# wdmwhh/MRefSR

Measured on AMD Instinct MI355X. Metric: 4x SR Mpix/sec, 5-ref 160x160->640x640; PSNR within 0.01 dB of ref, higher is better.
Workload: dtype f32

## Files before the change

### mrefsr_amd/csrc/mrattn_conv.hip

```cpp
#include "conv_common.h"

namespace {
using namespace mrefsr_conv;

constexpr int TG = 5;
constexpr int TR = 8, TW = 32;
constexpr int PH = TR + 2, PW = TW + 2, NPIX = PH * PW;
constexpr int QPL = NPIX * 16;
constexpr int TPL = 4 * QPL;
constexpr int NPIECE = NPIX * 4;
constexpr int NPK = (NPIECE + 255) / 256;
constexpr int NJ = 4;
constexpr int LDS_RAW = TG * TPL;
constexpr int LDS_BYTES = LDS_RAW + TR * TW * 4 + 64 + 16;

struct BlendArgs {
    const float *refs, *prob, *bias, *in_amax;
    const unsigned short *wp;
    const unsigned int *valid_bits;
    int *range_flag;
    float *out;
    int N, T, H, W, ncb;
    float out_scale;
};

template <int C, bool MASKED>
__global__ __launch_bounds__(256) void mrattn_blend_conv_kernel(const BlendArgs A)
{
    constexpr int NCH = C / KC, COUT = 2 * C, TAPS = 9, NW = 3;
    extern __shared__ __align__(16) unsigned char smem[];
    float *psum = reinterpret_cast<float *>(smem + LDS_RAW);
    int *tlist = reinterpret_cast<int *>(smem + LDS_RAW + TR * TW * 4);
    const int tid = threadIdx.x, lane = tid & 63, wv = tid >> 6, l31 = lane & 31, kh = lane >> 5;
    const int H = A.H, W = A.W, T = A.T, N = A.N;
    const int tx_n = (W + TW - 1) / TW, ty_n = (H + TR - 1) / TR;
    const unsigned int lin = blockIdx.x, seq = lin >> 3;
    const int cbk = (int)(seq % (unsigned)A.ncb);
    const long tile = (long)(seq / (unsigned)A.ncb) * 8 + (lin & 7u);
    if (tile >= (long)tx_n * ty_n * N) return;
    const int n = (int)(tile / (tx_n * ty_n)), trem = (int)(tile - (long)n * (tx_n * ty_n));
    const int y0 = (trem / tx_n) * TR, x0 = (trem % tx_n) * TW;

    if (tid == 0) {
        const unsigned int vb = MASKED ? A.valid_bits[n] : 0xffffffffu;
        int c = 0;
        for (int t = 0; t < T; ++t)
            if ((vb >> t) & 1u) tlist[c++] = t;
        tlist[16] = c;
    }
    float in_s = 1.f, oscale = A.out_scale;
    amax_scale<14>(A.in_amax, in_s, oscale);
    __syncthreads();
    const int total = __builtin_amdgcn_readfirstlane(tlist[16]);
    const int n_grp = (total + TG - 1) / TG, n_it = NCH * n_grp;

    const float *prow[2];
    bool pok[2];
#pragma unroll
    for (int m = 0; m < 2; ++m) {
        const int gy = y0 + wv * 2 + m, gx = x0 + l31;
        pok[m] = gy < H && gx < W;
        prow[m] = A.prob + (((size_t)n * H + (gy < H ? gy : H - 1)) * W + (gx < W ? gx : W - 1)) * T;
        float s = 0.f;
        for (int k = 0; k < total; ++k) s += prow[m][__builtin_amdgcn_readfirstlane(tlist[k])];
        if (kh == 0) psum[(wv * 2 + m) * TW + l31] = pok[m] ? s : 0.f;
    }

    f32x16 acc[2][NJ];
#pragma unroll
    for (int m = 0; m < 2; ++m)
#pragma unroll
        for (int j = 0; j < NJ; ++j)
#pragma unroll
            for (int e = 0; e < 16; ++e) acc[m][j][e] = 0.f;

    int goff[NPK], loff[NPK];
    unsigned int in_map = 0u, in_tile = 0u;
#pragma unroll
    for (int k = 0; k < NPK; ++k) {
        const int i = tid + k * 256;
        const int p = i >> 2, q = i & 3;
        const int py = p / PW, px = p - py * PW;
        const int gy = y0 + py - 1, gx = x0 + px - 1;
        const bool tile = i < NPIECE, ok = tile && gy >= 0 && gy < H && gx >= 0 && gx < W;
        goff[k] = ok ? (gy * W + gx) * C + 4 * q : 0;
        loff[k] = q * QPL + p * 16;
        in_map |= (ok ? 1u : 0u) << k, in_tile |= (tile ? 1u : 0u) << k;
    }
    float4 pf[TG][NPK];
    auto fetch = [&](const int it) {
        const int ch = it / n_grp, g = it - ch * n_grp;
        const int cnt = total - g * TG < TG ? total - g * TG : TG;
#pragma unroll
        for (int tg = 0; tg < TG; ++tg)
            if (tg < cnt) {
                const int t = __builtin_amdgcn_readfirstlane(tlist[g * TG + tg]);
                const float *base = A.refs + ((size_t)t * N + n) * H * W * C + ch * KC;
#pragma unroll
                for (int k = 0; k < NPK; ++k)
                    pf[tg][k] = ((in_map >> k) & 1u) ? *reinterpret_cast<const float4 *>(base + goff[k]) : make_float4(0.f, 0.f, 0.f, 0.f);
            }
    };
    if (n_it) fetch(0);

    const unsigned short *wlane = A.wp + (size_t)l31 * KC + kh * 8;
    auto bload = [&](const int lin, u32x4 (&b)[NJ][2]) {
#pragma unroll
        for (int j = 0; j < NJ; ++j)
#pragma unroll
            for (int sp = 0; sp < 2; ++sp)
                b[j][sp] = *reinterpret_cast<const u32x4 *>(wlane + ((((size_t)(cbk * 2 + (j >> 1)) * NCH * TAPS + lin) * NW + sp) * NB + (j & 1) * 32) * KC);
    };

    bool bad = false;
    float pr[2][TG];
    for (int it = 0; it < n_it; ++it) {
        const int ch = it / n_grp, g = it - ch * n_grp;
        const int cnt = total - g * TG < TG ? total - g * TG : TG;
        if (it) __syncthreads();
#pragma unroll
        for (int tg = 0; tg < TG; ++tg)
            if (tg < cnt) {
#pragma unroll
                for (int k = 0; k < NPK; ++k) {
                    float4 v = pf[tg][k];
                    v.x *= in_s, v.y *= in_s, v.z *= in_s, v.w *= in_s;
                    bad = bad || !(fmaxf(fmaxf(fabsf(v.x), fabsf(v.y)), fmaxf(fabsf(v.z), fabsf(v.w))) <= 65000.f);
                    if ((in_tile >> k) & 1u) *reinterpret_cast<float4 *>(smem + tg * TPL + loff[k]) = v;
                }
            }
        __syncthreads();
        if (it + 1 < n_it) fetch(it + 1);
        if (n_grp > 1 || it == 0) {
#pragma unroll
            for (int m = 0; m < 2; ++m)
#pragma unroll
                for (int k = 0; k < TG; ++k) pr[m][k] = (k < cnt && pok[m]) ? prow[m][__builtin_amdgcn_readfirstlane(tlist[g * TG + k])] : 0.f;
        }
        u32x4 b[NJ][2];
        bload(ch * TAPS, b);
#pragma nounroll
        for (int tap = 0; tap < TAPS; ++tap) {
            const int dy = (tap * 11) >> 5, dx = tap - 3 * dy;
            u32x4 bn[NJ][2];
            if (tap + 1 < TAPS) bload(ch * TAPS + tap + 1, bn);
#pragma unroll
            for (int m = 0; m < 2; ++m) {
                const unsigned char *sp = smem + (2 * kh) * QPL + ((wv * 2 + m + dy) * PW + l31 + dx) * 16;
                float u[8];
#pragma unroll
                for (int c = 0; c < 8; ++c) u[c] = 0.f;
#pragma unroll
                for (int k = 0; k < TG; ++k)
                    if (k < cnt) {
                        const float4 s0 = *reinterpret_cast<const float4 *>(sp + k * TPL);
                        const float4 s1 = *reinterpret_cast<const float4 *>(sp + k * TPL + QPL);
                        const float w = pr[m][k];
                        u[0] = fmaf(w, s0.x, u[0]), u[1] = fmaf(w, s0.y, u[1]), u[2] = fmaf(w, s0.z, u[2]), u[3] = fmaf(w, s0.w, u[3]);
                        u[4] = fmaf(w, s1.x, u[4]), u[5] = fmaf(w, s1.y, u[5]), u[6] = fmaf(w, s1.z, u[6]), u[7] = fmaf(w, s1.w, u[7]);
                    }
                u32x4 ah, al;
#pragma unroll
                for (int c = 0; c < 4; ++c) {
                    unsigned int h, l;
                    split_scaled(u[2 * c], u[2 * c + 1], h, l);
                    ah[c] = h, al[c] = l;
                }
#pragma unroll
                for (int j = 0; j < NJ; ++j) acc[m][j] = mma16(ah, b[j][1], acc[m][j]);
#pragma unroll
                for (int j = 0; j < NJ; ++j) acc[m][j] = mma16(al, scale_wh(b[j][0]), acc[m][j]);
#pragma unroll
                for (int j = 0; j < NJ; ++j) acc[m][j] = mma16(ah, b[j][0], acc[m][j]);
            }
            if (tap + 1 < TAPS) {
#pragma unroll
                for (int j = 0; j < NJ; ++j) b[j][0] = bn[j][0], b[j][1] = bn[j][1];
            }
        }
    }
    if (bad && A.range_flag) atomicOr(A.range_flag, 1);
    __syncthreads();

#pragma unroll
    for (int m = 0; m < 2; ++m) {
        const int gy = y0 + wv * 2 + m;
        if (gy >= H) continue;
#pragma unroll
        for (int j = 0; j < NJ; ++j) {
            const int co = cbk * (NJ * 32) + j * 32 + l31;
            const float bv = A.bias ? A.bias[co] : 0.f;
            float *orow = A.out + (((size_t)n * H + gy) * W) * COUT + co;
#pragma unroll
            for (int e = 0; e < 16; ++e) {
                const int x = (e & 3) + 8 * (e >> 2) + 4 * kh, gx = x0 + x;
                if (gx < W) orow[(size_t)gx * COUT] = acc[m][j][e] * oscale + bv * psum[(wv * 2 + m) * TW + x];
            }
        }
    }
}

template <int C, bool MASKED> int launch_blend_c(const BlendArgs &a, const dim3 grid, hipStream_t st)
{
    static unsigned long long attr_done = 0;
    if (mrefsr::first_use_on_device(attr_done)) {
        const hipError_t e = hipFuncSetAttribute(reinterpret_cast<const void *>(&mrattn_blend_conv_kernel<C, MASKED>),
                                                 hipFuncAttributeMaxDynamicSharedMemorySize, LDS_BYTES);
        if (e != hipSuccess) {
            attr_done = 0;
            (void)hipGetLastError();
            return mrefsr::fail(MREFSR_E_LAUNCH, "mrattn_blend_conv: %d bytes of dynamic LDS refused: %s", LDS_BYTES, hipGetErrorString(e));
        }
    }
    hipLaunchKernelGGL((mrattn_blend_conv_kernel<C, MASKED>), grid, dim3(256), LDS_BYTES, st, a);
    return mrefsr::check_launch("mrattn_blend_conv");
}

template <bool MASKED> int launch_blend(const BlendArgs &a, int C, hipStream_t st)
{
    const long tiles = (long)((a.W + TW - 1) / TW) * ((a.H + TR - 1) / TR) * a.N;
    const dim3 grid((unsigned)(((tiles + 7) / 8) * 8 * a.ncb));
    if (C == 64) return launch_blend_c<64, MASKED>(a, grid, st);
    if (C == 128) return launch_blend_c<128, MASKED>(a, grid, st);
    return launch_blend_c<256, MASKED>(a, grid, st);
}

}

MREFSR_EXPORT int mrefsr_mrattn_blend_conv_f32(const float *refs, const float *prob, const void *packed, const float *bias,
                                               const uint32_t *valid_bits, const float *in_amax, int *range_flag, float *out, int N, int T,
                                               int H, int W, int C, float wscale, mrefsr_stream_t stream)
{
    MREFSR_REQUIRE(refs && prob && packed && out, "mrattn_blend_conv: null pointer");
    MREFSR_REQUIRE(N > 0 && T > 0 && T <= 16 && H > 0 && W > 0, "mrattn_blend_conv: N=%d T=%d H=%d W=%d (T <= 16)", N, T, H, W);
    MREFSR_REQUIRE((int64_t)((W + TW - 1) / TW) * ((H + TR - 1) / TR) * N < (int64_t)1 << 28, "mrattn_blend_conv: N=%d H=%d W=%d (too many tiles)", N, H, W);
    MREFSR_REQUIRE((int64_t)H * W * 256 < (int64_t)1 << 31, "mrattn_blend_conv: H=%d W=%d (32-bit offsets inside a map)", H, W);
    MREFSR_REQUIRE(wscale > 0.f, "mrattn_blend_conv: wscale=%g", (double)wscale);
    if (C != 64 && C != 128 && C != 256)
        return mrefsr::fail(MREFSR_E_UNSUPPORTED, "mrattn_blend_conv: c=%d (64, 128 or 256: the three MRAPAFusion heads)", C);
    BlendArgs a;
    a.refs = refs, a.prob = prob, a.bias = bias, a.in_amax = in_amax;
    a.wp = reinterpret_cast<const unsigned short *>(packed);
    a.valid_bits = valid_bits, a.range_flag = range_flag, a.out = out;
    a.N = N, a.T = T, a.H = H, a.W = W, a.ncb = 2 * C / (NJ * 32);
    a.out_scale = 1.0f / wscale;
    return valid_bits ? launch_blend<true>(a, C, (hipStream_t)stream) : launch_blend<false>(a, C, (hipStream_t)stream);
}
```

Baseline: 17.25.

## Halve blend-conv tile rows, software-pipeline taps, and specialise on reference count

Tile height drops from 8 to 4 rows, so each wave handles one output row. Launch bounds now ask for two blocks per CU, with a static assert that LDS fits. The tap loop is fully unrolled and software-pipelined: the next tap's LDS reads, probability blend and hi/lo split are interleaved between the current tap's MFMAs using sched_barriers. The per-reference count is made a compile-time constant for 1 to 5 references. Input scaling moves into the probability weights, the range check becomes an integer max on the centre tap compared against a precomputed bound, and out-of-image halo is zeroed once rather than on every pass. The risks are more halo overhead per output pixel from the smaller tile, more register pressure, and rounding differences from folding the scale into the weights.

```diff
diff --git a/mrefsr_amd/csrc/mrattn_conv.hip b/mrefsr_amd/csrc/mrattn_conv.hip
--- a/mrefsr_amd/csrc/mrattn_conv.hip
+++ b/mrefsr_amd/csrc/mrattn_conv.hip
@@ -1,10 +1,12 @@
+#include <type_traits>
+
 #include "conv_common.h"
 
 namespace {
 using namespace mrefsr_conv;
 
 constexpr int TG = 5;
-constexpr int TR = 8, TW = 32;
+constexpr int TR = 4, TW = 32;
 constexpr int PH = TR + 2, PW = TW + 2, NPIX = PH * PW;
 constexpr int QPL = NPIX * 16;
 constexpr int TPL = 4 * QPL;
@@ -13,6 +15,7 @@
 constexpr int NJ = 4;
 constexpr int LDS_RAW = TG * TPL;
 constexpr int LDS_BYTES = LDS_RAW + TR * TW * 4 + 64 + 16;
+static_assert(2 * LDS_BYTES <= 160 * 1024, "two blocks per CU");
 
 struct BlendArgs {
     const float *refs, *prob, *bias, *in_amax;
@@ -25,7 +28,7 @@
 };
 
 template <int C, bool MASKED>
-__global__ __launch_bounds__(256) void mrattn_blend_conv_kernel(const BlendArgs A)
+__global__ __launch_bounds__(256, 2) void mrattn_blend_conv_kernel(const BlendArgs A)
 {
     constexpr int NCH = C / KC, COUT = 2 * C, TAPS = 9, NW = 3;
     extern __shared__ __align__(16) unsigned char smem[];
@@ -50,151 +53,180 @@
     }
     float in_s = 1.f, oscale = A.out_scale;
     amax_scale<14>(A.in_amax, in_s, oscale);
+    const unsigned int guard_bits = __float_as_uint(fminf(65000.f / in_s, 3.4028234664e38f));
     __syncthreads();
     const int total = __builtin_amdgcn_readfirstlane(tlist[16]);
     const int n_grp = (total + TG - 1) / TG, n_it = NCH * n_grp;
 
-    const float *prow[2];
-    bool pok[2];
-#pragma unroll
-    for (int m = 0; m < 2; ++m) {
-        const int gy = y0 + wv * 2 + m, gx = x0 + l31;
-        pok[m] = gy < H && gx < W;
-        prow[m] = A.prob + (((size_t)n * H + (gy < H ? gy : H - 1)) * W + (gx < W ? gx : W - 1)) * T;
+    const int gy_w = y0 + wv, gx_w = x0 + l31;
+    const bool pok = gy_w < H && gx_w < W;
+    const float *prow = A.prob + (((size_t)n * H + (gy_w < H ? gy_w : H - 1)) * W + (gx_w < W ? gx_w : W - 1)) * T;
+    {
         float s = 0.f;
-        for (int k = 0; k < total; ++k) s += prow[m][__builtin_amdgcn_readfirstlane(tlist[k])];
-        if (kh == 0) psum[(wv * 2 + m) * TW + l31] = pok[m] ? s : 0.f;
-    }
-
-    f32x16 acc[2][NJ];
-#pragma unroll
-    for (int m = 0; m < 2; ++m)
-#pragma unroll
-        for (int j = 0; j < NJ; ++j)
-#pragma unroll
-            for (int e = 0; e < 16; ++e) acc[m][j][e] = 0.f;
-
-    int goff[NPK], loff[NPK];
-    unsigned int in_map = 0u, in_tile = 0u;
+        for (int k = 0; k < total; ++k) s += prow[__builtin_amdgcn_readfirstlane(tlist[k])];
+        if (kh == 0) psum[wv * TW + l31] = pok ? s : 0.f;
+    }
+
+    f32x16 acc[NJ];
+#pragma unroll
+    for (int j = 0; j < NJ; ++j)
+#pragma unroll
+        for (int e = 0; e < 16; ++e) acc[j][e] = 0.f;
+
+    unsigned int goff[NPK], loff[NPK];
+    bool in_map[NPK];
 #pragma unroll
     for (int k = 0; k < NPK; ++k) {
         const int i = tid + k * 256;
         const int p = i >> 2, q = i & 3;
         const int py = p / PW, px = p - py * PW;
         const int gy = y0 + py - 1, gx = x0 + px - 1;
-        const bool tile = i < NPIECE, ok = tile && gy >= 0 && gy < H && gx >= 0 && gx < W;
-        goff[k] = ok ? (gy * W + gx) * C + 4 * q : 0;
-        loff[k] = q * QPL + p * 16;
-        in_map |= (ok ? 1u : 0u) << k, in_tile |= (tile ? 1u : 0u) << k;
-    }
-    float4 pf[TG][NPK];
-    auto fetch = [&](const int it) {
-        const int ch = it / n_grp, g = it - ch * n_grp;
-        const int cnt = total - g * TG < TG ? total - g * TG : TG;
-#pragma unroll
-        for (int tg = 0; tg < TG; ++tg)
-            if (tg < cnt) {
-                const int t = __builtin_amdgcn_readfirstlane(tlist[g * TG + tg]);
-                const float *base = A.refs + ((size_t)t * N + n) * H * W * C + ch * KC;
-#pragma unroll
-                for (int k = 0; k < NPK; ++k)
-                    pf[tg][k] = ((in_map >> k) & 1u) ? *reinterpret_cast<const float4 *>(base + goff[k]) : make_float4(0.f, 0.f, 0.f, 0.f);
+        const bool tile = i < NPIECE;
+        in_map[k] = tile && gy >= 0 && gy < H && gx >= 0 && gx < W;
+        goff[k] = in_map[k] ? (unsigned int)((gy * W + gx) * C + 4 * q) : 0u;
+        loff[k] = tile ? q * QPL + p * 16 : 0;
+        if (tile && !in_map[k]) {
+#pragma unroll
+            for (int tg = 0; tg < TG; ++tg) *reinterpret_cast<float4 *>(smem + tg * TPL + loff[k]) = make_float4(0.f, 0.f, 0.f, 0.f);
+        }
+    }
+
+    const unsigned int wl_off = (unsigned int)(l31 * KC + kh * 8) * 2u;
+    auto bload = [&](const int lin, u32x4 (&b)[NJ][2]) {
+#pragma unroll
+        for (int j = 0; j < NJ; ++j)
+#pragma unroll
+            for (int sp = 0; sp < 2; ++sp) {
+                const unsigned short *wu = A.wp + (((size_t)(cbk * 2 + (j >> 1)) * NCH * TAPS + lin) * NW * NB) * KC;
+                b[j][sp] = *reinterpret_cast<const u32x4 *>(reinterpret_cast<const unsigned char *>(wu) + wl_off + (sp * NB + (j & 1) * 32) * KC * 2);
             }
     };
-    if (n_it) fetch(0);
-
-    const unsigned short *wlane = A.wp + (size_t)l31 * KC + kh * 8;
-    auto bload = [&](const int lin, u32x4 (&b)[NJ][2]) {
-#pragma unroll
-        for (int j = 0; j < NJ; ++j)
-#pragma unroll
-            for (int sp = 0; sp < 2; ++sp)
-                b[j][sp] = *reinterpret_cast<const u32x4 *>(wlane + ((((size_t)(cbk * 2 + (j >> 1)) * NCH * TAPS + lin) * NW + sp) * NB + (j & 1) * 32) * KC);
+
+    unsigned int worst = 0u;
+    const unsigned char *sp0 = smem + (2 * kh) * QPL + (wv * PW + l31) * 16;
+    auto taps = [&](auto cnt_c, const int cnt, const int ch, u32x4 (&b)[2][NJ][2], const float (&pr)[TG]) {
+        constexpr int CNT = decltype(cnt_c)::value ? decltype(cnt_c)::value : TG;
+        constexpr bool FIXED = decltype(cnt_c)::value != 0;
+        f32x4 s[CNT][2];
+        float u[8];
+        u32x4 ah, al, nh, nl, w2[NJ];
+        auto rd = [&](const int tap) {
+            const unsigned char *sp = sp0 + (((tap * 11) >> 5) * (PW - 3) + tap) * 16;
+#pragma unroll
+            for (int k = 0; k < CNT; ++k)
+                if (FIXED || k < cnt) {
+                    s[k][0] = *reinterpret_cast<const f32x4 *>(sp + k * TPL);
+                    s[k][1] = *reinterpret_cast<const f32x4 *>(sp + k * TPL + QPL);
+                }
+        };
+        auto chain = [&](const int k, const bool centre) {
+            if (!FIXED && k >= cnt) return;
+            const float w = pr[k];
+#pragma unroll
+            for (int c = 0; c < 4; ++c) u[c] = fmaf(w, s[k][0][c], k ? u[c] : 0.f), u[4 + c] = fmaf(w, s[k][1][c], k ? u[4 + c] : 0.f);
+            if (centre) {
+                const unsigned int m = 0x7fffffffu;
+#pragma unroll
+                for (int h = 0; h < 2; ++h)
+                    worst = max(worst, max(max(__float_as_uint(s[k][h][0]) & m, __float_as_uint(s[k][h][1]) & m),
+                                           max(__float_as_uint(s[k][h][2]) & m, __float_as_uint(s[k][h][3]) & m)));
+            }
+        };
+        auto split = [&](const int c) {
+            unsigned int h, l;
+            split_scaled(u[2 * c], u[2 * c + 1], h, l);
+            nh[c] = h, nl[c] = l;
+        };
+        rd(0);
+#pragma unroll
+        for (int k = 0; k < CNT; ++k) chain(k, false);
+#pragma unroll
+        for (int c = 0; c < 4; ++c) split(c);
+        ah = nh, al = nl;
+#pragma unroll
+        for (int tap = 0; tap < TAPS; ++tap) {
+            const bool more = tap + 1 < TAPS;
+            u32x4 (&bc)[NJ][2] = b[tap & 1];
+            if (more) {
+                bload(ch * TAPS + tap + 1, b[(tap + 1) & 1]);
+                rd(tap + 1);
+            }
+            __builtin_amdgcn_sched_barrier(0);
+#pragma unroll
+            for (int sl = 0; sl < 12; ++sl) {
+                const int j = sl & 3;
+                if (sl < 4) acc[j] = mma16(ah, bc[j][1], acc[j]);
+                else if (sl < 8) acc[j] = mma16(al, w2[j], acc[j]);
+                else acc[j] = mma16(ah, bc[j][0], acc[j]);
+                if (sl < 2) w2[2 * sl] = scale_wh(bc[2 * sl][0]), w2[2 * sl + 1] = scale_wh(bc[2 * sl + 1][0]);
+                if (more) {
+                    if (sl >= 2 && sl - 2 < CNT) chain(sl - 2, tap + 1 == 4);
+                    if (sl >= 7 && sl < 11) split(sl - 7);
+                }
+                __builtin_amdgcn_sched_barrier(0);
+            }
+            if (more) ah = nh, al = nl;
+        }
     };
-
-    bool bad = false;
-    float pr[2][TG];
-    for (int it = 0; it < n_it; ++it) {
-        const int ch = it / n_grp, g = it - ch * n_grp;
-        const int cnt = total - g * TG < TG ? total - g * TG : TG;
-        if (it) __syncthreads();
-#pragma unroll
-        for (int tg = 0; tg < TG; ++tg)
-            if (tg < cnt) {
-#pragma unroll
-                for (int k = 0; k < NPK; ++k) {
-                    float4 v = pf[tg][k];
-                    v.x *= in_s, v.y *= in_s, v.z *= in_s, v.w *= in_s;
-                    bad = bad || !(fmaxf(fmaxf(fabsf(v.x), fabsf(v.y)), fmaxf(fabsf(v.z), fabsf(v.w))) <= 65000.f);
-                    if ((in_tile >> k) & 1u) *reinterpret_cast<float4 *>(smem + tg * TPL + loff[k]) = v;
-                }
-            }
-        __syncthreads();
-        if (it + 1 < n_it) fetch(it + 1);
-        if (n_grp > 1 || it == 0) {
-#pragma unroll
-            for (int m = 0; m < 2; ++m)
-#pragma unroll
-                for (int k = 0; k < TG; ++k) pr[m][k] = (k < cnt && pok[m]) ? prow[m][__builtin_amdgcn_readfirstlane(tlist[g * TG + k])] : 0.f;
-        }
-        u32x4 b[NJ][2];
-        bload(ch * TAPS, b);
-#pragma nounroll
-        for (int tap = 0; tap < TAPS; ++tap) {
-            const int dy = (tap * 11) >> 5, dx = tap - 3 * dy;
-            u32x4 bn[NJ][2];
-            if (tap + 1 < TAPS) bload(ch * TAPS + tap + 1, bn);
-#pragma unroll
-            for (int m = 0; m < 2; ++m) {
-                const unsigned char *sp = smem + (2 * kh) * QPL + ((wv * 2 + m + dy) * PW + l31 + dx) * 16;
-                float u[8];
-#pragma unroll
-                for (int c = 0; c < 8; ++c) u[c] = 0.f;
-#pragma unroll
-                for (int k = 0; k < TG; ++k)
-                    if (k < cnt) {
-                        const float4 s0 = *reinterpret_cast<const float4 *>(sp + k * TPL);
-                        const float4 s1 = *reinterpret_cast<const float4 *>(sp + k * TPL + QPL);
-                        const float w = pr[m][k];
-                        u[0] = fmaf(w, s0.x, u[0]), u[1] = fmaf(w, s0.y, u[1]), u[2] = fmaf(w, s0.z, u[2]), u[3] = fmaf(w, s0.w, u[3]);
-                        u[4] = fmaf(w, s1.x, u[4]), u[5] = fmaf(w, s1.y, u[5]), u[6] = fmaf(w, s1.z, u[6]), u[7] = fmaf(w, s1.w, u[7]);
+    float pr[TG];
+    auto passes = [&](auto cnt_c) {
+        for (int it = 0; it < n_it; ++it) {
+            const int ch = it / n_grp, g = it - ch * n_grp;
+            const int cnt = total - g * TG < TG ? total - g * TG : TG;
+            {
+                f32x4 pf[TG][NPK];
+#pragma unroll
+                for (int tg = 0; tg < TG; ++tg)
+                    if (tg < cnt) {
+                        const int t = __builtin_amdgcn_readfirstlane(tlist[g * TG + tg]);
+                        const float *base = A.refs + ((size_t)t * N + n) * H * W * C + ch * KC;
+#pragma unroll
+                        for (int k = 0; k < NPK; ++k) pf[tg][k] = *reinterpret_cast<const f32x4 *>(base + goff[k]);
+                    } else {
+#pragma unroll
+                        for (int k = 0; k < NPK; ++k) pf[tg][k] = f32x4{0.f, 0.f, 0.f, 0.f};
                     }
-                u32x4 ah, al;
-#pragma unroll
-                for (int c = 0; c < 4; ++c) {
-                    unsigned int h, l;
-                    split_scaled(u[2 * c], u[2 * c + 1], h, l);
-                    ah[c] = h, al[c] = l;
-                }
-#pragma unroll
-                for (int j = 0; j < NJ; ++j) acc[m][j] = mma16(ah, b[j][1], acc[m][j]);
-#pragma unroll
-                for (int j = 0; j < NJ; ++j) acc[m][j] = mma16(al, scale_wh(b[j][0]), acc[m][j]);
-#pragma unroll
-                for (int j = 0; j < NJ; ++j) acc[m][j] = mma16(ah, b[j][0], acc[m][j]);
-            }
-            if (tap + 1 < TAPS) {
-#pragma unroll
-                for (int j = 0; j < NJ; ++j) b[j][0] = bn[j][0], b[j][1] = bn[j][1];
-            }
-        }
-    }
-    if (bad && A.range_flag) atomicOr(A.range_flag, 1);
+                if (it) __syncthreads();
+#pragma unroll
+                for (int tg = 0; tg < TG; ++tg)
+                    if (tg < cnt) {
+#pragma unroll
+                        for (int k = 0; k < NPK; ++k)
+                            if (in_map[k]) *reinterpret_cast<f32x4 *>(smem + tg * TPL + loff[k]) = pf[tg][k];
+                    }
+            }
+            __builtin_amdgcn_sched_barrier(0);
+            if (n_grp > 1 || it == 0) {
+#pragma unroll
+                for (int k = 0; k < TG; ++k) pr[k] = (k < cnt && pok) ? prow[__builtin_amdgcn_readfirstlane(tlist[g * TG + k])] * in_s : 0.f;
+            }
+            u32x4 b[2][NJ][2];
+            bload(ch * TAPS, b[0]);
+            __syncthreads();
+            taps(cnt_c, cnt, ch, b, pr);
+        }
+    };
+    switch (total <= TG ? total : 0) {
+    case 1: passes(std::integral_constant<int, 1>{}); break;
+    case 2: passes(std::integral_constant<int, 2>{}); break;
+    case 3: passes(std::integral_constant<int, 3>{}); break;
+    case 4: passes(std::integral_constant<int, 4>{}); break;
+    case 5: passes(std::integral_constant<int, 5>{}); break;
+    default: passes(std::integral_constant<int, 0>{}); break;
+    }
+    if (worst > guard_bits && A.range_flag) atomicOr(A.range_flag, 1);
     __syncthreads();
 
-#pragma unroll
-    for (int m = 0; m < 2; ++m) {
-        const int gy = y0 + wv * 2 + m;
-        if (gy >= H) continue;
+    if (gy_w < H) {
 #pragma unroll
         for (int j = 0; j < NJ; ++j) {
             const int co = cbk * (NJ * 32) + j * 32 + l31;
             const float bv = A.bias ? A.bias[co] : 0.f;
-            float *orow = A.out + (((size_t)n * H + gy) * W) * COUT + co;
+            float *orow = A.out + (((size_t)n * H + gy_w) * W) * COUT + co;
 #pragma unroll
             for (int e = 0; e < 16; ++e) {
                 const int x = (e & 3) + 8 * (e >> 2) + 4 * kh, gx = x0 + x;
-                if (gx < W) orow[(size_t)gx * COUT] = acc[m][j][e] * oscale + bv * psum[(wv * 2 + m) * TW + x];
+                if (gx < W) orow[(size_t)gx * COUT] = acc[j][e] * oscale + bv * psum[wv * TW + x];
             }
         }
     }
```

New measurement: 17.70 (median of 6 runs). 2.6% higher.
